# Tongdongq/darwin-gpu

Measured on AMD Instinct MI355X. Metric: GACT GCUPS (DP cells/s) on ~10 kb PacBio-shape reads, higher is better.
Workload: dtype int16x2 (packed); 1 GPU; ecoli10x_self_overlap; tile_size=320, tile_overlap=120, scoring=+1/-1/-1/-1, reads=4642, bases=48503677, candidates=65766, tiles=2185214, parallelism=candidates dealt round-robin over 1 GPU(s), slots_in_flight=4, passes_in_this_process=127, arch=gfx950:sramecc+:xnack-

## Files before the change

darwin-gpu_amd/csrc/gact_lin.hpp:

```cpp
#pragma once

#include "gact_p16s.hpp"

namespace gact {

#ifndef GACT_LIN_MAX3
#define GACT_LIN_MAX3 1
#endif
constexpr int kLinFloor = GACT_LIN_MAX3 ? 1024 : 0;
__host__ __device__ constexpr int lin_base(int g) { return kLinFloor + 40 * (-g) + 8; }
__device__ __forceinline__ uint32_t vconst(uint32_t s)
{
    uint32_t r;
    asm volatile("s_nop 1\n\tv_mov_b32 %0, %1" : "=v"(r) : "s"(s));
    return r;
}

__host__ inline bool p16_lin_ok(int tile, int match, int mismatch, int open, int ext)
{
    const long long steps = (long long)tile + 4 * kGroup + 64 + 48;
    return open == ext && mismatch == ext && ext <= 0 && match >= 0 &&
           p16_tagged_ok(tile, match, mismatch, open, ext) &&
           4 * ((long long)match * (tile + 2) + (long long)(-ext) * steps + kLinFloor) + 3 <= 30000 && match - ext <= 63;
}

__device__ __forceinline__ uint32_t pk_mad4v(uint32_t a, uint32_t v_c)
{
    uint32_t r;
    asm("v_pk_mad_u16 %0, %1, 4, %2 op_sel_hi:[1,0,1]" : "=v"(r) : "v"(a), "v"(v_c));
    return r;
}
__device__ __forceinline__ uint32_t pk_max3f(uint32_t a, uint32_t b, uint32_t c)
{
    uint32_t r;
    asm("v_pk_maximum3_f16 %0, %1, %2, %3" : "=v"(r) : "v"(a), "v"(b), "v"(c));
    return r;
}
__device__ __forceinline__ uint32_t andn_or(uint32_t a, uint32_t b, uint32_t c)
{
    uint32_t r;
    asm("v_bitop3_b32 %0, %1, %2, %3 bitop3:0xba" : "=v"(r) : "v"(a), "v"(b), "v"(c));
    return r;
}
__device__ __forceinline__ uint32_t pk_ashr2(uint32_t a)
{
    uint32_t r;
    asm("v_pk_ashrrev_i16 %0, 2, %1 op_sel_hi:[0,1]" : "=v"(r) : "v"(a));
    return r;
}


template <int CW> struct LinWords {
    static constexpr int kWords = (CW + 1) / 2;
    static constexpr int kUint4 = (kWords + 3) / 4;
};
template <int NW, int LANES, class Fix>
__device__ __forceinline__ void lin_flush(const uint32_t (&acc)[2 * NW], uint4 *qA, uint4 *qB, Fix fix, const bool storeA, const bool storeB)
{
    constexpr int QD = (NW + 3) / 4;
    uint32_t wa[QD * 4], wb[QD * 4];
#pragma unroll
    for (int n = 0; n < QD * 4; n++) {
        wa[n] = n < NW ? fix(__builtin_amdgcn_perm(acc[n < NW ? 2 * n + 1 : 0], acc[n < NW ? 2 * n : 0], 0x05040100u)) : 0u;
        wb[n] = n < NW ? fix(__builtin_amdgcn_perm(acc[n < NW ? 2 * n + 1 : 0], acc[n < NW ? 2 * n : 0], 0x07060302u)) : 0u;
    }
    if (storeA) {
#pragma unroll
        for (int q = 0; q < QD; q++) qA[q * kWsRow] = make_uint4(wa[4 * q], wa[4 * q + 1], wa[4 * q + 2], wa[4 * q + 3]);
    }
    if (storeB) {
#pragma unroll
        for (int q = 0; q < QD; q++) qB[q * kWsRow] = make_uint4(wb[4 * q], wb[4 * q + 1], wb[4 * q + 2], wb[4 * q + 3]);
    }
}

constexpr int kLinBandDefault = 48, kLinBandMin = 24, kLinBandQuantum = 1;
struct LinBand {
    int lo[2], hi[2];
    bool full[2];
    __device__ __forceinline__ bool store(int h, int first, int last) const { return full[h] | ((last >= lo[h]) & (first <= hi[h])); }
};
__device__ __forceinline__ void lin_band_range(LinBand &b, int h, int T_end, int behind, int dj_min, int dj_max, int band, bool full)
{
    b.full[h] = full | (band <= 0);
    b.lo[h] = T_end - behind - dj_max - band;
    b.hi[h] = dj_max < 0 ? -0x40000000 : T_end - behind - imax(dj_min, 0) + band;
}

template <int C1, int C2>
__device__ __forceinline__ uint32_t dp_pass_lin_split(const P16Consts &kc, const int gl,
                                                      const uint16_t *__restrict__ ref16,
                                                      const uint32_t (&qb)[C1 + C2],
                                                      const int T_end, const int tB,
                                                      uint32_t *__restrict__ wsA, uint32_t *__restrict__ wsB,
                                                      const int band, const bool fullA, const bool fullB,
                                                      const uint32_t *lut_lds)
{
    constexpr int CT = C1 + C2;
    constexpr int NW = LinWords<C2>::kWords, QD = LinWords<C2>::kUint4;
    constexpr int LAG = kGroup;
    const int g = (int)(int16_t)(kc.ext & 0xffffu);
    const uint32_t gv = vconst(kc.next), g4v = vconst(kc.next4), c3v = vconst(kc.c3), onev = vconst(kc.one),
                   dtv = vconst(kc.next4 + kc.tag1),
                   c2v = vconst(kc.tag2);
    uint32_t Z1 = pk2(lin_base(g) + gl * g), Z2 = pk2(lin_base(g) + (gl + LAG) * g);
    uint32_t G[CT];
    uint32_t acc[2 * NW];
#pragma unroll
    for (int c = 0; c < CT; c++) G[c] = c < C1 ? Z1 : Z2;
#pragma unroll
    for (int c = 0; c < 2 * NW; c++) acc[c] = 0;
    uint32_t H1 = Z1, H2 = Z2;
    uint32_t Hdiag1 = Z1, Hdiag2 = Z2;

    typedef __attribute__((address_space(3))) const uint8_t LdsByte;
    typedef __attribute__((address_space(3))) const uint32_t LdsWord;
    LdsByte *const lut_plain = (LdsByte *)lut_lds, *const lut_tagged = (LdsByte *)(lut_lds + 1);
    auto row = [](LdsByte *table, uint32_t stream_byte) { return *(LdsWord *)(table + stream_byte); };
    LdsByte *rp = (LdsByte *)(ref16 + (1 - LAG));
    uint32_t rb1 = row(lut_plain, rp[2 * LAG]), rb1b = row(lut_plain, rp[2 * LAG + 1]);
    uint32_t rb2 = row(lut_plain, rp[0]), rb2b = row(lut_plain, rp[1]);
    rp += 2;

#define GACT_SB() __builtin_amdgcn_sched_barrier(0)
    uint32_t sb1 = 0, sb1b = 0, sb2 = 0, sb2b = 0;
    auto ask_bytes = [&](const bool r1, const bool r2) {
        if (r2) { sb2 = rp[0]; sb2b = rp[1]; }
        if (r1) { sb1 = rp[2 * LAG]; sb1b = rp[2 * LAG + 1]; }
        rp += 2;
    };
    auto ask_rows = [&](const bool r1, const bool r2, const bool tag2) {
        if (r1) { rb1 = row(lut_plain, sb1); rb1b = row(lut_plain, sb1b); }
        if (r2) { rb2 = row(tag2 ? lut_tagged : lut_plain, sb2); rb2b = row(tag2 ? lut_tagged : lut_plain, sb2b); }
    };
    auto upper_all = [&](uint32_t (&U)[CT], const bool tag2, const uint32_t Zr2) {
        uint32_t P[CT];
#pragma unroll
        for (int c = 0; c < CT; c++) P[c] = __builtin_amdgcn_perm(c < C1 ? rb1b : rb2b, c < C1 ? rb1 : rb2, qb[c]);
        GACT_SB();
#pragma unroll
        for (int c = 0; c < CT; c++) U[c] = (c == 0 ? Hdiag1 : c == C1 ? Hdiag2 : G[c - 1]) + P[c];
        ask_rows(true, true, tag2);
        GACT_SB();
        if (GACT_LIN_MAX3) {
#pragma unroll
            for (int c = 0; c < CT; c++)
                U[c] = pk_max3f(U[c], c < C1 ? Z1 : Zr2, G[c]);
        } else {
#pragma unroll
            for (int c = 0; c < CT; c++) U[c] = pk_max(U[c], c < C1 ? Z1 : Zr2);
            GACT_SB();
#pragma unroll
            for (int c = 0; c < CT; c++) U[c] = pk_max(U[c], G[c]);
        }
        GACT_SB();
    };

    auto step = [&]() {
        ask_bytes(true, true);
        Z1 += gv; Z2 += gv;
        const uint32_t Hl1 = (uint32_t)dpp_row_shr1((int)H1, (int)Z1);
        const uint32_t Hl2 = (uint32_t)dpp_row_shr1((int)H2, dpp_row_ror1((int)H1));
        uint32_t U[CT];
        upper_all(U, false, Z2);
        Hdiag1 = Hl1; Hdiag2 = Hl2;
        uint32_t Ha = Hl1, Hb = Hl2;
        static_assert(C2 >= C1, "region 2 is the longer chain");
#pragma unroll
        for (int c = 0; c < C1; c++) {
            const uint32_t Da = Ha - gv, Db = Hb - gv;
            GACT_SB();
            G[c] = pk_max(U[c], Da); G[C1 + c] = pk_max(U[C1 + c], Db);
            GACT_SB();
            Ha = G[c]; Hb = G[C1 + c];
        }
#pragma unroll
        for (int c = 2 * C1; c < CT; c++) { G[c] = pk_max(U[c], Hb - gv); Hb = G[c]; }
        H1 = Ha; H2 = Hb;
    };
    auto step_r1 = [&]() {
        ask_bytes(true, false);
        Z1 += gv; Z2 += gv;
        const uint32_t Hl1 = (uint32_t)dpp_row_shr1((int)H1, (int)Z1);
        uint32_t P[C1], U[C1];
#pragma unroll
        for (int c = 0; c < C1; c++) P[c] = __builtin_amdgcn_perm(rb1b, rb1, qb[c]);
        GACT_SB();
#pragma unroll
        for (int c = 0; c < C1; c++) U[c] = (c == 0 ? Hdiag1 : G[c - 1]) + P[c];
        ask_rows(true, false, false);
        GACT_SB();
#pragma unroll
        for (int c = 0; c < C1; c++) U[c] = GACT_LIN_MAX3 ? pk_max3f(U[c], Z1, G[c]) : pk_max(pk_max(U[c], Z1), G[c]);
        GACT_SB();
        Hdiag1 = Hl1;
        uint32_t Ha = Hl1;
#pragma unroll
        for (int c = 0; c < C1; c++) { G[c] = pk_max(U[c], Ha - gv); Ha = G[c]; }
        H1 = Ha;
    };

    uint32_t Z24 = 0;
    auto step_tagged = [&]() {
        ask_bytes(true, true);
        Z1 += gv; Z24 += g4v;
        const uint32_t Hl1 = (uint32_t)dpp_row_shr1((int)H1, (int)Z1);
        const uint32_t Hl2 = (uint32_t)dpp_row_shr1((int)H2, dpp_row_ror1((int)pk_mad4v(H1, c2v)));
        uint32_t U[CT];
        upper_all(U, true, Z24);
        Hdiag1 = Hl1; Hdiag2 = Hl2;
        uint32_t Ha = Hl1, Hb = Hl2;
        uint32_t tprev = 0;
#pragma unroll
        for (int c = 0; c < C2; c++) {
            const bool both = c < C1;
            uint32_t Da = 0;
            const uint32_t Db = Hb - dtv;
            if (both) Da = Ha - gv;
            GACT_SB();
            const uint32_t Hp = pk_max(U[C1 + c], Db);
            if (both) { G[c] = pk_max(U[c], Da); Ha = G[c]; }
            if (c > 0) acc[c - 1] = pk_shl_add4(acc[c - 1], tprev);
            GACT_SB();
            G[C1 + c] = andn_or(Hp, c3v, c2v);
            tprev = Hp & c3v;
            GACT_SB();
            Hb = G[C1 + c];
        }
        acc[C2 - 1] = pk_shl_add4(acc[C2 - 1], tprev);
        H1 = Ha; H2 = Hb;
    };
    auto step_tagged_r2 = [&]() {
        ask_bytes(false, true);
        Z24 += g4v;
        const uint32_t Hl2 = (uint32_t)dpp_row_shr1((int)H2, dpp_row_ror1((int)pk_mad4v(H1, c2v)));
        uint32_t P[C2], U[C2];
#pragma unroll
        for (int c = 0; c < C2; c++) P[c] = __builtin_amdgcn_perm(rb2b, rb2, qb[C1 + c]);
        GACT_SB();
#pragma unroll
        for (int c = 0; c < C2; c++) U[c] = (c == 0 ? Hdiag2 : G[C1 + c - 1]) + P[c];
        ask_rows(false, true, true);
        GACT_SB();
#pragma unroll
        for (int c = 0; c < C2; c++) U[c] = GACT_LIN_MAX3 ? pk_max3f(U[c], Z24, G[C1 + c]) : pk_max(pk_max(U[c], Z24), G[C1 + c]);
        GACT_SB();
        Hdiag2 = Hl2;
        uint32_t Hb = Hl2;
        uint32_t tprev = 0;
#pragma unroll
        for (int c = 0; c < C2; c++) {
            const uint32_t Db = Hb - dtv;
            GACT_SB();
            const uint32_t Hp = pk_max(U[c], Db);
            if (c > 0) acc[c - 1] = pk_shl_add4(acc[c - 1], tprev);
            GACT_SB();
            G[C1 + c] = andn_or(Hp, c3v, c2v);
            tprev = Hp & c3v;
            GACT_SB();
            Hb = G[C1 + c];
        }
        acc[C2 - 1] = pk_shl_add4(acc[C2 - 1], tprev);
        H2 = Hb;
    };
#undef GACT_SB
    auto enter_tagged = [&]() {
#pragma unroll
        for (int c = C1; c < CT; c++) G[c] = pk_mad4v(G[c], c2v);
        H2 = pk_mad4v(H2, c2v);
        Hdiag2 = pk_mad4v(Hdiag2, c2v);
        Z24 = pk_mad4v(Z2, c3v);
        rb2 = row(lut_tagged, rp[-2]); rb2b = row(lut_tagged, rp[-1]);
    };

    int t = 1;
    for (const int tP = imin(LAG, imin(tB - 1, T_end)); t <= tP; t++) step_r1();
    if (t > 1) {
#pragma unroll
        for (int c = C1; c < CT; c++) G[c] = Z2;
        H2 = Z2; Hdiag2 = Z2;
        rb2 = row(lut_plain, rp[-2]); rb2b = row(lut_plain, rp[-1]);
    }
    const int tU = imin(tB - 1, T_end);
    for (; t + 1 <= tU; t += 2) { step(); step(); }
    if (t <= tU) { step(); t++; }
    const bool tagged = t <= T_end;
    if (tagged) enter_tagged();
    uint4 *qA = reinterpret_cast<uint4 *>(wsA) + gl;
    uint4 *qB = reinterpret_cast<uint4 *>(wsB) + gl;
    LinBand bd;
    {
        const int q1 = (band >> 16) - 1, b = band & 0xffff;
        const int u_lo = kGroup - 1 - (gl & ~q1), u_hi = kGroup - 1 - (gl | q1);
        LinBand lo_, hi_;
        lin_band_range(lo_, 0, T_end, u_lo, C2 * u_lo, C2 * u_lo + C2 - 1, b, fullA);
        lin_band_range(hi_, 0, T_end, u_hi, C2 * u_hi, C2 * u_hi + C2 - 1, b, fullA);
        bd.lo[0] = bd.lo[1] = lo_.lo[0]; bd.hi[0] = bd.hi[1] = hi_.hi[0];
        bd.full[0] = fullA | (b <= 0); bd.full[1] = fullB | (b <= 0);
    }
    int k = 0;
    while (t + 7 <= T_end && t <= T_end - LAG) {
#pragma unroll
        for (int s8 = 0; s8 < 8; s8++, t++) step_tagged();
        k += 8;
        lin_flush<NW, kGroup>(acc, qA, qB, [](uint32_t w) { return w; }, bd.store(0, t - 8, t - 1), bd.store(1, t - 8, t - 1));
        qA += QD * kWsRow;
        qB += QD * kWsRow;
    }
    while (t + 7 <= T_end) {
#pragma unroll
        for (int s8 = 0; s8 < 8; s8++, t++) step_tagged_r2();
        k += 8;
        lin_flush<NW, kGroup>(acc, qA, qB, [](uint32_t w) { return w; }, bd.store(0, t - 8, t - 1), bd.store(1, t - 8, t - 1));
        qA += QD * kWsRow;
        qB += QD * kWsRow;
    }
    for (; t <= T_end - LAG; t++, k++) step_tagged();
    for (; t <= T_end; t++, k++) step_tagged_r2();
    if (k & 7) {
        const int sh = 2 * (8 - (k & 7));
        lin_flush<NW, kGroup>(acc, qA, qB, [sh](uint32_t w) { return ((w & 0xffffu) << sh & 0xffffu) | ((w >> 16) << sh << 16); },
                              bd.store(0, t - (k & 7), t - 1), bd.store(1, t - (k & 7), t - 1));
    }
    return tagged ? pk_ashr2(pk_sub(H2 | kc.c3, Z24)) : pk_sub(H2, Z2);
}

template <int C, int LANES, bool AMAX>
__device__ __forceinline__ uint32_t dp_pass_lin(const P16Consts &kc, const int gl,
                                                const uint16_t *__restrict__ ref16,
                                                const uint32_t (&qb)[C],
                                                const int T_end, const int tB,
                                                uint32_t *__restrict__ wsA, uint32_t *__restrict__ wsB,
                                                const int cqA, const int cqB, const int (*RQ)[2], P16Best *pb,
                                                const int col_from, const int band, const int QA, const int QB,
                                                const bool fullA, const bool fullB)
{
    constexpr int NW = LinWords<C>::kWords, QD = LinWords<C>::kUint4;
    const bool store = AMAX || gl * C + C >= col_from;
    LinBand bd;
    {
        const int q1 = AMAX ? 0 : (band >> 16) - 1, b = AMAX ? 0 : band & 0xffff;
        const int g_lo = gl & ~q1, g_hi = gl | q1;
        LinBand lo_, hi_;
        lin_band_range(lo_, 0, T_end, (imax(QA, 1) - 1) / C - g_lo, QA - g_lo * C - C, QA - g_lo * C - 1, b, fullA);
        lin_band_range(lo_, 1, T_end, (imax(QB, 1) - 1) / C - g_lo, QB - g_lo * C - C, QB - g_lo * C - 1, b, fullB);
        lin_band_range(hi_, 0, T_end, (imax(QA, 1) - 1) / C - g_hi, QA - g_hi * C - C, QA - g_hi * C - 1, b, fullA);
        lin_band_range(hi_, 1, T_end, (imax(QB, 1) - 1) / C - g_hi, QB - g_hi * C - C, QB - g_hi * C - 1, b, fullB);
        bd = lo_;
        bd.hi[0] = hi_.hi[0] < 0 ? (lo_.hi[0] < 0 ? lo_.hi[0] : T_end) : hi_.hi[0];
        bd.hi[1] = hi_.hi[1] < 0 ? (lo_.hi[1] < 0 ? lo_.hi[1] : T_end) : hi_.hi[1];
    }
    static_assert(!AMAX || LANES == kGroup, "first tiles run on the 16-lane layout");
    const int g = (int)(int16_t)(kc.ext & 0xffffu);
    const uint32_t gv = vconst(kc.next), g4v = vconst(kc.next4), c3v = vconst(kc.c3), onev = vconst(kc.one),
                   dtv = vconst(kc.next4 + kc.tag1),
                   c2v = vconst(kc.tag2), lut1v = vconst(0x01010101u);
    uint32_t Z = pk2(lin_base(g) + gl * g);
    uint32_t G[C];
    uint32_t acc[2 * NW];
#pragma unroll
    for (int c = 0; c < C; c++) G[c] = Z;
#pragma unroll
    for (int c = 0; c < 2 * NW; c++) acc[c] = 0;
    uint32_t G_last = Z, Hdiag = Z;

    uint32_t bk[AMAX ? C : 1];
    int lane_best[2] = {-1, -1};
    uint32_t col_x0 = 0;
    int t_first = 0, rows[2] = {0, 0};
    if (AMAX) {
#pragma unroll
        for (int c = 0; c < C; c++) bk[c] = 0xffffffffu;
        const int ncA = imin(imax(RQ[0][1] - gl * C, 0), C), ncB = imin(imax(RQ[1][1] - gl * C, 0), C);
        col_x0 = ((uint32_t)(-ncA) & 0xffffu) | ((uint32_t)(-ncB) << 16);
        t_first = gl + 1;
        rows[0] = RQ[0][0]; rows[1] = RQ[1][0];
    }

    auto lut = [&](uint32_t amount) { return kc.dsub >> (amount & 31u); };
    auto lut4 = [&](uint32_t amount) { return kc.dsub4 >> (amount & 31u); };
    uint32_t lutA = 0, lutB = 0;
    { const uint32_t w = ref16[1]; lutA = lut(w & 0xffu); lutB = lut(w >> 8); }

    auto shr1 = [](uint32_t v, uint32_t old) {
        return (uint32_t)(LANES == 32 ? dpp_shr1_32((int)v, (int)old) : dpp_row_shr1((int)v, (int)old));
    };

#define GACT_SB() __builtin_amdgcn_sched_barrier(0)
    auto upper_all = [&](uint32_t (&U)[C], const bool tag2, const uint32_t Zr) {
        uint32_t P[C];
#pragma unroll
        for (int c = 0; c < C; c++) P[c] = __builtin_amdgcn_perm(lutB, lutA, qb[c]);
        GACT_SB();
#pragma unroll
        for (int c = 0; c < C; c++) U[c] = (c == 0 ? Hdiag : G[c - 1]) + P[c];
        (void)tag2;
        GACT_SB();
        if (GACT_LIN_MAX3) {
#pragma unroll
            for (int c = 0; c < C; c++) U[c] = pk_max3f(U[c], Zr, G[c]);
        } else {
#pragma unroll
            for (int c = 0; c < C; c++) U[c] = pk_max(U[c], Zr);
            GACT_SB();
#pragma unroll
            for (int c = 0; c < C; c++) U[c] = pk_max(U[c], G[c]);
        }
        GACT_SB();
    };

    auto step = [&](const int t) {
        const uint32_t w_next = ref16[t + 1];
        Z += gv;
        const uint32_t Hl0 = shr1(G_last, Z);
        uint32_t U[C];
        upper_all(U, false, Z);
        Hdiag = Hl0;
        uint32_t Hl = Hl0;
#pragma unroll
        for (int c = 0; c < C; c++) { G[c] = pk_max(U[c], Hl - gv); Hl = G[c]; }
        G_last = Hl;
        lutA = lut(w_next & 0xffu); lutB = lut(w_next >> 8);
    };

    uint32_t Z4 = 0, Z8 = 0;
    auto step_tagged = [&](const int t) {
        const uint32_t w_next = ref16[t + 1];
        Z4 += g4v;
        uint32_t key_c = 0;
        if (AMAX) {
            Z8 += g4v + g4v;
            const uint32_t sidx = (uint32_t)(t - tB) & 7u, row0 = (uint32_t)(t - t_first);
            const uint32_t ka = row0 < (uint32_t)rows[0] ? sidx : ((uint32_t)kKeyBias & 0xffffu);
            const uint32_t kb = row0 < (uint32_t)rows[1] ? sidx : ((uint32_t)kKeyBias & 0xffffu);
            key_c = pk_sub(ka | (kb << 16), Z8);
        }
        const uint32_t Hl0 = shr1(G_last, Z4 - onev);
        uint32_t U[C];
        upper_all(U, true, Z4);
        Hdiag = Hl0;
        uint32_t Hl = Hl0, tprev = 0;
#pragma unroll
        for (int c = 0; c < C; c++) {
            const uint32_t Db = Hl - dtv;
            GACT_SB();
            const uint32_t Hp = pk_max(U[c], Db);
            if (c > 0) {
                acc[c - 1] = pk_shl_add4(acc[c - 1], tprev);
                if (AMAX) bk[c - 1] = pk_max(bk[c - 1], pk_mad_vvv(G[c - 1], kc.tag2, key_c));
            }
            GACT_SB();
            G[c] = andn_or(Hp, c3v, c2v);
            tprev = Hp & c3v;
            GACT_SB();
            Hl = G[c];
        }
        acc[C - 1] = pk_shl_add4(acc[C - 1], tprev);
        if (AMAX) bk[C - 1] = pk_max(bk[C - 1], pk_mad_vvv(G[C - 1], kc.tag2, key_c));
        G_last = Hl;
        lutA = lut4(w_next & 0xffu) + lut1v; lutB = lut4(w_next >> 8) + lut1v;
    };
#undef GACT_SB
    auto enter_tagged = [&]() {
#pragma unroll
        for (int c = 0; c < C; c++) G[c] = pk_mad4v(G[c], c2v);
        G_last = pk_mad4v(G_last, c2v);
        Hdiag = pk_mad4v(Hdiag, c2v);
        Z4 = pk_mad4v(Z, c3v);
        Z8 = Z4 + Z4 - c2v;
        lutA = (lutA << 2) + lut1v; lutB = (lutB << 2) + lut1v;
    };

    auto fold = [&](const int kblk) {
        uint32_t m = 0xffffffffu, rel = 0, x = col_x0;
#pragma unroll
        for (int c = 0; c < C; c++) {
            const uint32_t v = pk_sign(x);
            x = pk_add(x, kc.one);
            const uint32_t key = pk_mad_m1(v, pk_add(bk[AMAX ? c : 0], kc.one));
            const uint32_t keep = pk_sign(pk_sub(key, m));
            rel = pk_mad_m1(keep, rel);
            m = pk_max(m, key);
            bk[AMAX ? c : 0] = 0xffffffffu;
        }
#pragma unroll
        for (int h = 0; h < 2; h++) {
            const int m16 = (int)(m << (16 - 16 * h)) >> 16;
            const int col = ((int)(rel << (16 - 16 * h)) >> 16) + C;
            const int rec = ((m16 >> 3) << 15) | ((kblk + (m16 & 7)) << 5) | col;
            lane_best[h] = imax(lane_best[h], m16 < 0 ? -1 : rec);
        }
    };

    int t = 1;
    for (; t < tB && t <= T_end; t++) step(t);
    const bool tagged = t <= T_end;
    if (tagged) enter_tagged();
    uint4 *qA = reinterpret_cast<uint4 *>(wsA) + gl;
    uint4 *qB = reinterpret_cast<uint4 *>(wsB) + gl;
    int k = 0;
    while (t + 7 <= T_end) {
        for (int s8 = 0; s8 < 8; s8++, t++) step_tagged(t);
        k += 8;
        lin_flush<NW, LANES>(acc, qA, qB, [](uint32_t w) { return w; }, store && bd.store(0, t - 8, t - 1), store && bd.store(1, t - 8, t - 1));
        qA += QD * kWsRow;
        qB += QD * kWsRow;
        if (AMAX) fold(k - 8);
    }
    for (; t <= T_end; t++, k++) step_tagged(t);
    if (AMAX) {
        if (k & 7) fold(k & ~7);
#pragma unroll
        for (int h = 0; h < 2; h++) {
            const int rec = lane_best[h];
            int best = 0, bi = 0, bj = 0;
            if (rec >= 0) {
                best = rec >> 15;
                bi = tB + ((rec >> 5) & 1023) - gl;
                bj = gl * C + (rec & 31) + 1;
            }
#pragma unroll
            for (int mm = 1; mm < kGroup; mm <<= 1) {
                const int ob = __shfl_xor(best, mm, kGroup);
                const int oi = __shfl_xor(bi, mm, kGroup);
                const int oj = __shfl_xor(bj, mm, kGroup);
                const bool take = (ob > best) | ((ob == best) & ((oi > bi) | ((oi == bi) & (oj > bj))));
                best = take ? ob : best;
                bi = take ? oi : bi;
                bj = take ? oj : bj;
            }
            pb->best[h] = best; pb->bi[h] = bi; pb->bj[h] = bj;
        }
    }
    if (k & 7) {
        const int sh = 2 * (8 - (k & 7));
        lin_flush<NW, LANES>(acc, qA, qB, [sh](uint32_t w) { return ((w & 0xffffu) << sh & 0xffffu) | ((w >> 16) << sh << 16); },
                             store && bd.store(0, t - (k & 7), t - 1), store && bd.store(1, t - (k & 7), t - 1));
    }
    if (AMAX) return 0;
    uint32_t ga = G[0], gb = G[0];
#pragma unroll
    for (int c = 1; c < C; c++) { ga = (c == cqA) ? G[c] : ga; gb = (c == cqB) ? G[c] : gb; }
    const uint32_t pick = __builtin_amdgcn_perm(gb, ga, 0x07060100u);
    return tagged ? pk_ashr2(pk_sub(pick | kc.c3, Z4)) : pk_sub(pick, Z);
}

struct WideLayoutLin : UniformLayout<10, 32, true> {
    static constexpr int kWalkFmt = 3, kWalkQuads = LinWords<10>::kUint4;
#ifndef GACT_WALK_SPAN
#define GACT_WALK_SPAN 16
#endif
    static constexpr int kWalkSpan = GACT_WALK_SPAN;
#ifndef GACT_WIDE_LIN_BLOCKS
#define GACT_WIDE_LIN_BLOCKS 3
#endif
    static constexpr int kBlocksPerCu = GACT_WIDE_LIN_BLOCKS;
    static constexpr bool kEndAligned = true;
    template <bool RAW>
    __device__ static uint32_t pass(const P16Consts &kc, int gl, const uint16_t *ref16, const uint32_t (&qb)[10], int T_end,
                                    int tB, uint32_t *wsA, uint32_t *wsB, const PairTile &pt)
    {
        static_assert(!RAW, "the linear-gap pass reads 2-bit sets");
        return dp_pass_lin<10, 32, false>(kc, gl, ref16, qb, T_end, tB, wsA, wsB, (imax(pt.Q[0], 1) - 1) % 10,
                                          (imax(pt.Q[1], 1) - 1) % 10, nullptr, nullptr, pt.col_from, pt.band, pt.Q[0], pt.Q[1],
                                          pt.full[0], pt.full[1]);
    }
    __device__ static int fin_lane(int Q) { return (imax(Q, 1) - 1) / 10; }
};

#ifndef GACT_LIN_BLOCKS_PER_CU
#define GACT_LIN_BLOCKS_PER_CU 3
#endif
template <int C1, int C2> struct SplitLayoutLin : SplitLayout<C1, C2, true> {
    static constexpr int kBlocksPerCu = GACT_LIN_BLOCKS_PER_CU;
    static constexpr int kWalkFmt = 3, kWalkQuads = LinWords<C2>::kUint4;
    static constexpr int kWalkSpan = GACT_WALK_SPAN;
    static constexpr bool kEndAligned = true;
    static constexpr int kLutWords = kLinLutWords;
    using Base = SplitLayout<C1, C2, true>;
    template <bool RAW>
    __device__ static void load(const SeqSetDev &rs, const SeqSetDev &qf, const SeqSetDev &qr,
                                const PairTile &pt, int gl, uint8_t *ref8, uint8_t *q8, uint32_t (&qb)[C1 + C2], uint32_t *stage)
    {
        static_assert(!RAW, "the linear-gap pass reads 2-bit sets");
        load_pair_packed<C1 + C2, kGroup, typename Base::Cols, true, kLinPadRow>(rs, qf, qr, pt, gl, ref8, Base::G::kRefBytes, Base::G::kRow0, q8,
                                                                                 Base::G::kTileMax, qb, stage, typename Base::Cols{});
    }
    template <bool RAW>
    __device__ static uint32_t pass(const P16Consts &kc, int gl, const uint16_t *ref16, const uint32_t (&qb)[C1 + C2],
                                    int T_end, int tB, uint32_t *wsA, uint32_t *wsB, const PairTile &pt)
    {
        static_assert(!RAW, "the linear-gap pass reads 2-bit sets");
        return dp_pass_lin_split<C1, C2>(kc, gl, ref16, qb, T_end, tB, wsA, wsB, pt.band, pt.full[0], pt.full[1], pt.lut);
    }
    __device__ static int fin_lane(int Q) { (void)Q; return kGroup - 1; }
};

template <int C1, int C2> struct SplitLayoutLinTeam : SplitLayoutLin<C1, C2> {
    static constexpr bool kTeamWalk = true;
};

}
```

Before: 8961 GCUPS.

## Pack traceback bits of column pairs with byte perms in tagged linear-gap pass

In the blocked tagged steps of the split linear-gap pass, the 2-bit traceback codes for adjacent column pairs are merged with a v_perm into one word and accumulated per pair. This replaces a per-column shift-add into the accumulator array, and the flush now does a single perm per output word. The intent is to cut VALU work on the inner DP recurrence's side path. It also adds wrappers that can switch pk_max/pk_sub and the inline asm helpers to compiler builtins, off by default. The cost is more complex position-templated code, more live registers and a new static_assert requiring an odd C2.

```diff
diff --git a/darwin-gpu_amd/csrc/gact_lin.hpp b/darwin-gpu_amd/csrc/gact_lin.hpp
--- a/darwin-gpu_amd/csrc/gact_lin.hpp
+++ b/darwin-gpu_amd/csrc/gact_lin.hpp
@@ -24,6 +24,26 @@
            4 * ((long long)match * (tile + 2) + (long long)(-ext) * steps + kLinFloor) + 3 <= 30000 && match - ext <= 63;
 }
 
+#ifndef GACT_LIN_BUILTINS
+#define GACT_LIN_BUILTINS 0
+#endif
+typedef short LinS2 __attribute__((ext_vector_type(2)));
+__device__ __forceinline__ uint32_t lin_max(uint32_t a, uint32_t b)
+{
+#if GACT_LIN_BUILTINS
+    return __builtin_bit_cast(uint32_t, __builtin_elementwise_max(__builtin_bit_cast(LinS2, a), __builtin_bit_cast(LinS2, b)));
+#else
+    return pk_max(a, b);
+#endif
+}
+__device__ __forceinline__ uint32_t lin_sub(uint32_t a, uint32_t b)
+{
+#if GACT_LIN_BUILTINS
+    return __builtin_bit_cast(uint32_t, (LinS2)(__builtin_bit_cast(LinS2, a) - __builtin_bit_cast(LinS2, b)));
+#else
+    return pk_sub(a, b);
+#endif
+}
 __device__ __forceinline__ uint32_t pk_mad4v(uint32_t a, uint32_t v_c)
 {
     uint32_t r;
@@ -38,17 +58,32 @@
 }
 __device__ __forceinline__ uint32_t andn_or(uint32_t a, uint32_t b, uint32_t c)
 {
+#if GACT_LIN_BUILTINS
+    return __builtin_amdgcn_bitop3_b32(a, b, c, 0xba);
+#else
     uint32_t r;
     asm("v_bitop3_b32 %0, %1, %2, %3 bitop3:0xba" : "=v"(r) : "v"(a), "v"(b), "v"(c));
     return r;
+#endif
 }
 __device__ __forceinline__ uint32_t pk_ashr2(uint32_t a)
 {
+#if GACT_LIN_BUILTINS
+    return __builtin_bit_cast(uint32_t, (LinS2)(__builtin_bit_cast(LinS2, a) >> (short)2));
+#else
     uint32_t r;
     asm("v_pk_ashrrev_i16 %0, 2, %1 op_sel_hi:[0,1]" : "=v"(r) : "v"(a));
     return r;
-}
-
+#endif
+}
+
+
+__device__ __forceinline__ uint32_t sconst_here(uint32_t lit)
+{
+    uint32_t r;
+    asm volatile("s_mov_b32 %0, %1" : "=s"(r) : "i"(lit));
+    return r;
+}
 
 template <int CW> struct LinWords {
     static constexpr int kWords = (CW + 1) / 2;
@@ -63,6 +98,36 @@
     for (int n = 0; n < QD * 4; n++) {
         wa[n] = n < NW ? fix(__builtin_amdgcn_perm(acc[n < NW ? 2 * n + 1 : 0], acc[n < NW ? 2 * n : 0], 0x05040100u)) : 0u;
         wb[n] = n < NW ? fix(__builtin_amdgcn_perm(acc[n < NW ? 2 * n + 1 : 0], acc[n < NW ? 2 * n : 0], 0x07060302u)) : 0u;
+    }
+    if (storeA) {
+#pragma unroll
+        for (int q = 0; q < QD; q++) qA[q * kWsRow] = make_uint4(wa[4 * q], wa[4 * q + 1], wa[4 * q + 2], wa[4 * q + 3]);
+    }
+    if (storeB) {
+#pragma unroll
+        for (int q = 0; q < QD; q++) qB[q * kWsRow] = make_uint4(wb[4 * q], wb[4 * q + 1], wb[4 * q + 2], wb[4 * q + 3]);
+    }
+}
+
+template <int S> struct LinPos { static constexpr int value = S; };
+constexpr int kLinTail = -1;
+constexpr uint32_t kLinPairSel = 0x06020400u;
+constexpr uint32_t kLinPairMask = 0x03030303u;
+constexpr uint32_t kLinFlushSelA = 0x05010400u;
+constexpr uint32_t kLinFlushSelB = 0x07030602u;
+template <int CW>
+__device__ __forceinline__ void lin_flush_groups(const uint32_t (&grp)[2 * (CW / 2)], const uint32_t odd, uint4 *qA, uint4 *qB,
+                                                 const bool storeA, const bool storeB)
+{
+    constexpr int NP = CW / 2, NW = LinWords<CW>::kWords, QD = LinWords<CW>::kUint4;
+    uint32_t wa[QD * 4], wb[QD * 4];
+    const uint32_t sA = sconst_here(kLinFlushSelA), sB = sconst_here(kLinFlushSelB);
+#pragma unroll
+    for (int n = 0; n < QD * 4; n++) {
+        wa[n] = n < NP ? __builtin_amdgcn_perm(grp[n < NP ? 2 * n : 0], grp[n < NP ? 2 * n + 1 : 0], sA)
+              : n < NW ? odd & 0xffffu : 0u;
+        wb[n] = n < NP ? __builtin_amdgcn_perm(grp[n < NP ? 2 * n : 0], grp[n < NP ? 2 * n + 1 : 0], sB)
+              : n < NW ? odd >> 16 : 0u;
     }
     if (storeA) {
 #pragma unroll
@@ -103,9 +168,11 @@
     const uint32_t gv = vconst(kc.next), g4v = vconst(kc.next4), c3v = vconst(kc.c3), onev = vconst(kc.one),
                    dtv = vconst(kc.next4 + kc.tag1),
                    c2v = vconst(kc.tag2);
+    const uint32_t psel = sconst_here(kLinPairSel);
     uint32_t Z1 = pk2(lin_base(g) + gl * g), Z2 = pk2(lin_base(g) + (gl + LAG) * g);
     uint32_t G[CT];
     uint32_t acc[2 * NW];
+    uint32_t grp[2 * (C2 / 2)], odd = 0;
 #pragma unroll
     for (int c = 0; c < CT; c++) G[c] = c < C1 ? Z1 : Z2;
 #pragma unroll
@@ -148,10 +215,10 @@
                 U[c] = pk_max3f(U[c], c < C1 ? Z1 : Zr2, G[c]);
         } else {
 #pragma unroll
-            for (int c = 0; c < CT; c++) U[c] = pk_max(U[c], c < C1 ? Z1 : Zr2);
-            GACT_SB();
-#pragma unroll
-            for (int c = 0; c < CT; c++) U[c] = pk_max(U[c], G[c]);
+            for (int c = 0; c < CT; c++) U[c] = lin_max(U[c], c < C1 ? Z1 : Zr2);
+            GACT_SB();
+#pragma unroll
+            for (int c = 0; c < CT; c++) U[c] = lin_max(U[c], G[c]);
         }
         GACT_SB();
     };
@@ -170,12 +237,12 @@
         for (int c = 0; c < C1; c++) {
             const uint32_t Da = Ha - gv, Db = Hb - gv;
             GACT_SB();
-            G[c] = pk_max(U[c], Da); G[C1 + c] = pk_max(U[C1 + c], Db);
+            G[c] = lin_max(U[c], Da); G[C1 + c] = lin_max(U[C1 + c], Db);
             GACT_SB();
             Ha = G[c]; Hb = G[C1 + c];
         }
 #pragma unroll
-        for (int c = 2 * C1; c < CT; c++) { G[c] = pk_max(U[c], Hb - gv); Hb = G[c]; }
+        for (int c = 2 * C1; c < CT; c++) { G[c] = lin_max(U[c], Hb - gv); Hb = G[c]; }
         H1 = Ha; H2 = Hb;
     };
     auto step_r1 = [&]() {
@@ -191,17 +258,24 @@
         ask_rows(true, false, false);
         GACT_SB();
 #pragma unroll
-        for (int c = 0; c < C1; c++) U[c] = GACT_LIN_MAX3 ? pk_max3f(U[c], Z1, G[c]) : pk_max(pk_max(U[c], Z1), G[c]);
+        for (int c = 0; c < C1; c++) U[c] = GACT_LIN_MAX3 ? pk_max3f(U[c], Z1, G[c]) : lin_max(lin_max(U[c], Z1), G[c]);
         GACT_SB();
         Hdiag1 = Hl1;
         uint32_t Ha = Hl1;
 #pragma unroll
-        for (int c = 0; c < C1; c++) { G[c] = pk_max(U[c], Ha - gv); Ha = G[c]; }
+        for (int c = 0; c < C1; c++) { G[c] = lin_max(U[c], Ha - gv); Ha = G[c]; }
         H1 = Ha;
     };
 
     uint32_t Z24 = 0;
-    auto step_tagged = [&]() {
+    static_assert(C2 >= 3 && (C2 & 1), "the last pair is filed while the unpaired slot is computed");
+    auto file_group = [&](const int S, const int c, const uint32_t x) {
+        uint32_t &r = grp[c - 2 + (S >> 2)];
+        r = (S & 3) ? pk_shl_add4(r, x) : x;
+    };
+    auto step_tagged = [&](auto pos) {
+        constexpr int S = decltype(pos)::value;
+        constexpr bool blk = S != kLinTail;
         ask_bytes(true, true);
         Z1 += gv; Z24 += g4v;
         const uint32_t Hl1 = (uint32_t)dpp_row_shr1((int)H1, (int)Z1);
@@ -210,27 +284,35 @@
         upper_all(U, true, Z24);
         Hdiag1 = Hl1; Hdiag2 = Hl2;
         uint32_t Ha = Hl1, Hb = Hl2;
-        uint32_t tprev = 0;
+        uint32_t tprev = 0, Hq = 0, x = 0;
 #pragma unroll
         for (int c = 0; c < C2; c++) {
             const bool both = c < C1;
+            const bool filed = blk && c >= 2 && !(c & 1);
             uint32_t Da = 0;
             const uint32_t Db = Hb - dtv;
             if (both) Da = Ha - gv;
-            GACT_SB();
-            const uint32_t Hp = pk_max(U[C1 + c], Db);
-            if (both) { G[c] = pk_max(U[c], Da); Ha = G[c]; }
-            if (c > 0) acc[c - 1] = pk_shl_add4(acc[c - 1], tprev);
+            if (filed) x &= kLinPairMask;
+            GACT_SB();
+            const uint32_t Hp = lin_max(U[C1 + c], Db);
+            if (both) { G[c] = lin_max(U[c], Da); Ha = G[c]; }
+            if (!blk && c > 0) acc[c - 1] = pk_shl_add4(acc[c - 1], tprev);
+            if (filed) file_group(S, c, x);
             GACT_SB();
             G[C1 + c] = andn_or(Hp, c3v, c2v);
-            tprev = Hp & c3v;
+            if (!blk || c == C2 - 1) tprev = Hp & c3v;
+            else if (c & 1) x = __builtin_amdgcn_perm(Hp, Hq, psel);
+            else Hq = Hp;
             GACT_SB();
             Hb = G[C1 + c];
         }
-        acc[C2 - 1] = pk_shl_add4(acc[C2 - 1], tprev);
+        if (!blk) acc[C2 - 1] = pk_shl_add4(acc[C2 - 1], tprev);
+        else odd = S ? pk_shl_add4(odd, tprev) : tprev;
         H1 = Ha; H2 = Hb;
     };
-    auto step_tagged_r2 = [&]() {
+    auto step_tagged_r2 = [&](auto pos) {
+        constexpr int S = decltype(pos)::value;
+        constexpr bool blk = S != kLinTail;
         ask_bytes(false, true);
         Z24 += g4v;
         const uint32_t Hl2 = (uint32_t)dpp_row_shr1((int)H2, dpp_row_ror1((int)pk_mad4v(H1, c2v)));
@@ -243,26 +325,34 @@
         ask_rows(false, true, true);
         GACT_SB();
 #pragma unroll
-        for (int c = 0; c < C2; c++) U[c] = GACT_LIN_MAX3 ? pk_max3f(U[c], Z24, G[C1 + c]) : pk_max(pk_max(U[c], Z24), G[C1 + c]);
+        for (int c = 0; c < C2; c++) U[c] = GACT_LIN_MAX3 ? pk_max3f(U[c], Z24, G[C1 + c]) : lin_max(lin_max(U[c], Z24), G[C1 + c]);
         GACT_SB();
         Hdiag2 = Hl2;
         uint32_t Hb = Hl2;
-        uint32_t tprev = 0;
+        uint32_t tprev = 0, Hq = 0, x = 0;
 #pragma unroll
         for (int c = 0; c < C2; c++) {
+            const bool filed = blk && c >= 2 && !(c & 1);
             const uint32_t Db = Hb - dtv;
-            GACT_SB();
-            const uint32_t Hp = pk_max(U[c], Db);
-            if (c > 0) acc[c - 1] = pk_shl_add4(acc[c - 1], tprev);
+            if (filed) x &= kLinPairMask;
+            GACT_SB();
+            const uint32_t Hp = lin_max(U[c], Db);
+            if (!blk && c > 0) acc[c - 1] = pk_shl_add4(acc[c - 1], tprev);
+            if (filed) file_group(S, c, x);
             GACT_SB();
             G[C1 + c] = andn_or(Hp, c3v, c2v);
-            tprev = Hp & c3v;
+            if (!blk || c == C2 - 1) tprev = Hp & c3v;
+            else if (c & 1) x = __builtin_amdgcn_perm(Hp, Hq, psel);
+            else Hq = Hp;
             GACT_SB();
             Hb = G[C1 + c];
         }
-        acc[C2 - 1] = pk_shl_add4(acc[C2 - 1], tprev);
+        if (!blk) acc[C2 - 1] = pk_shl_add4(acc[C2 - 1], tprev);
+        else odd = S ? pk_shl_add4(odd, tprev) : tprev;
         H2 = Hb;
     };
+#define GACT_LIN_BLOCK8(f) do { f(LinPos<0>{}); f(LinPos<1>{}); f(LinPos<2>{}); f(LinPos<3>{}); \
+                                f(LinPos<4>{}); f(LinPos<5>{}); f(LinPos<6>{}); f(LinPos<7>{}); } while (0)
 #undef GACT_SB
     auto enter_tagged = [&]() {
 #pragma unroll
@@ -300,29 +390,28 @@
     }
     int k = 0;
     while (t + 7 <= T_end && t <= T_end - LAG) {
-#pragma unroll
-        for (int s8 = 0; s8 < 8; s8++, t++) step_tagged();
-        k += 8;
-        lin_flush<NW, kGroup>(acc, qA, qB, [](uint32_t w) { return w; }, bd.store(0, t - 8, t - 1), bd.store(1, t - 8, t - 1));
+        GACT_LIN_BLOCK8(step_tagged);
+        t += 8; k += 8;
+        lin_flush_groups<C2>(grp, odd, qA, qB, bd.store(0, t - 8, t - 1), bd.store(1, t - 8, t - 1));
         qA += QD * kWsRow;
         qB += QD * kWsRow;
     }
     while (t + 7 <= T_end) {
-#pragma unroll
-        for (int s8 = 0; s8 < 8; s8++, t++) step_tagged_r2();
-        k += 8;
-        lin_flush<NW, kGroup>(acc, qA, qB, [](uint32_t w) { return w; }, bd.store(0, t - 8, t - 1), bd.store(1, t - 8, t - 1));
+        GACT_LIN_BLOCK8(step_tagged_r2);
+        t += 8; k += 8;
+        lin_flush_groups<C2>(grp, odd, qA, qB, bd.store(0, t - 8, t - 1), bd.store(1, t - 8, t - 1));
         qA += QD * kWsRow;
         qB += QD * kWsRow;
     }
-    for (; t <= T_end - LAG; t++, k++) step_tagged();
-    for (; t <= T_end; t++, k++) step_tagged_r2();
+#undef GACT_LIN_BLOCK8
+    for (; t <= T_end - LAG; t++, k++) step_tagged(LinPos<kLinTail>{});
+    for (; t <= T_end; t++, k++) step_tagged_r2(LinPos<kLinTail>{});
     if (k & 7) {
         const int sh = 2 * (8 - (k & 7));
         lin_flush<NW, kGroup>(acc, qA, qB, [sh](uint32_t w) { return ((w & 0xffffu) << sh & 0xffffu) | ((w >> 16) << sh << 16); },
                               bd.store(0, t - (k & 7), t - 1), bd.store(1, t - (k & 7), t - 1));
     }
-    return tagged ? pk_ashr2(pk_sub(H2 | kc.c3, Z24)) : pk_sub(H2, Z2);
+    return tagged ? pk_ashr2(lin_sub(H2 | kc.c3, Z24)) : lin_sub(H2, Z2);
 }
 
 template <int C, int LANES, bool AMAX>
@@ -401,10 +490,10 @@
             for (int c = 0; c < C; c++) U[c] = pk_max3f(U[c], Zr, G[c]);
         } else {
 #pragma unroll
-            for (int c = 0; c < C; c++) U[c] = pk_max(U[c], Zr);
-            GACT_SB();
-#pragma unroll
-            for (int c = 0; c < C; c++) U[c] = pk_max(U[c], G[c]);
+            for (int c = 0; c < C; c++) U[c] = lin_max(U[c], Zr);
+            GACT_SB();
+#pragma unroll
+            for (int c = 0; c < C; c++) U[c] = lin_max(U[c], G[c]);
         }
         GACT_SB();
     };
@@ -418,7 +507,7 @@
         Hdiag = Hl0;
         uint32_t Hl = Hl0;
 #pragma unroll
-        for (int c = 0; c < C; c++) { G[c] = pk_max(U[c], Hl - gv); Hl = G[c]; }
+        for (int c = 0; c < C; c++) { G[c] = lin_max(U[c], Hl - gv); Hl = G[c]; }
         G_last = Hl;
         lutA = lut(w_next & 0xffu); lutB = lut(w_next >> 8);
     };
@@ -433,7 +522,7 @@
             const uint32_t sidx = (uint32_t)(t - tB) & 7u, row0 = (uint32_t)(t - t_first);
             const uint32_t ka = row0 < (uint32_t)rows[0] ? sidx : ((uint32_t)kKeyBias & 0xffffu);
             const uint32_t kb = row0 < (uint32_t)rows[1] ? sidx : ((uint32_t)kKeyBias & 0xffffu);
-            key_c = pk_sub(ka | (kb << 16), Z8);
+            key_c = lin_sub(ka | (kb << 16), Z8);
         }
         const uint32_t Hl0 = shr1(G_last, Z4 - onev);
         uint32_t U[C];
@@ -444,10 +533,10 @@
         for (int c = 0; c < C; c++) {
             const uint32_t Db = Hl - dtv;
             GACT_SB();
-            const uint32_t Hp = pk_max(U[c], Db);
+            const uint32_t Hp = lin_max(U[c], Db);
             if (c > 0) {
                 acc[c - 1] = pk_shl_add4(acc[c - 1], tprev);
-                if (AMAX) bk[c - 1] = pk_max(bk[c - 1], pk_mad_vvv(G[c - 1], kc.tag2, key_c));
+                if (AMAX) bk[c - 1] = lin_max(bk[c - 1], pk_mad_vvv(G[c - 1], kc.tag2, key_c));
             }
             GACT_SB();
             G[c] = andn_or(Hp, c3v, c2v);
@@ -456,7 +545,7 @@
             Hl = G[c];
         }
         acc[C - 1] = pk_shl_add4(acc[C - 1], tprev);
-        if (AMAX) bk[C - 1] = pk_max(bk[C - 1], pk_mad_vvv(G[C - 1], kc.tag2, key_c));
+        if (AMAX) bk[C - 1] = lin_max(bk[C - 1], pk_mad_vvv(G[C - 1], kc.tag2, key_c));
         G_last = Hl;
         lutA = lut4(w_next & 0xffu) + lut1v; lutB = lut4(w_next >> 8) + lut1v;
     };
@@ -478,9 +567,9 @@
             const uint32_t v = pk_sign(x);
             x = pk_add(x, kc.one);
             const uint32_t key = pk_mad_m1(v, pk_add(bk[AMAX ? c : 0], kc.one));
-            const uint32_t keep = pk_sign(pk_sub(key, m));
+            const uint32_t keep = pk_sign(lin_sub(key, m));
             rel = pk_mad_m1(keep, rel);
-            m = pk_max(m, key);
+            m = lin_max(m, key);
             bk[AMAX ? c : 0] = 0xffffffffu;
         }
 #pragma unroll
@@ -542,7 +631,7 @@
 #pragma unroll
     for (int c = 1; c < C; c++) { ga = (c == cqA) ? G[c] : ga; gb = (c == cqB) ? G[c] : gb; }
     const uint32_t pick = __builtin_amdgcn_perm(gb, ga, 0x07060100u);
-    return tagged ? pk_ashr2(pk_sub(pick | kc.c3, Z4)) : pk_sub(pick, Z);
+    return tagged ? pk_ashr2(lin_sub(pick | kc.c3, Z4)) : lin_sub(pick, Z);
 }
 
 struct WideLayoutLin : UniformLayout<10, 32, true> {
```

Result: faster. 9215 GCUPS (median of 6 runs) (+2.8%).
